# SMSD75/Timetuning

Measured on AMD Instinct MI355X. Metric: clip-frames/sec, higher is better.
Workload: dtype f32-split(f16x3); 1 GPU; C2: dino-s16 full TimeT training step (fwd+bwd+AdamW), 4-frame 224x224 clips, 32 clips/GPU, 200 prototypes; clips_per_gpu=32, num_frames=4, num_clusters=200, global_batch=32, parallelism=dp1

## Files before the change

include/timetuning_hip.h:

```cpp
#ifndef TIMETUNING_HIP_H
#define TIMETUNING_HIP_H

#include <stddef.h>
#include <stdint.h>

#ifdef __cplusplus
extern "C" {
#endif

#define TT_OK 0
#define TT_EINVAL (-1)
#define TT_ELAUNCH (-2)
#define TT_EUNSUPPORTED (-3)

typedef void* tt_stream_t;

const char* tt_last_error(void);
int tt_abi_version(void);
int tt_set_tuning_knob(const char* name, int value);
int tt_tuning_knob_info(int index, const char** name, int* default_value, int* value);
int tt_device_info(char* name, int cap);

size_t tt_linear_ksplit_workspace_bytes(void);
int tt_linear_ksplit_workspace_init(void* workspace, size_t workspace_bytes, tt_stream_t stream);
// ... 41 lines not shown
int tt_patch_embed_fwd_planes(const float* img, const int32_t* frame_map, const void* w_planes, const float* bias, const float* cls,
                              const float* pos, float* tokens, int F, int C, int H, int W, int P, int D, void* workspace,
                              size_t workspace_bytes, tt_stream_t stream);

int tt_layernorm_fwd(const float* x, const float* gamma, const float* beta, float* y, float* mean, float* rstd,
                     int rows, int D, float eps, int skip_group, tt_stream_t stream);
size_t tt_amax_slot_bytes(void);
int tt_layernorm_bwd(const float* dy, const float* x, const float* gamma, const float* mean, const float* rstd,
                     float* dx, float* dgamma, float* dbeta, int rows, int D, int add_to_dx, int skip_group,
                     void* workspace, size_t workspace_bytes, float* amax_out, tt_stream_t stream);
size_t tt_layernorm_bwd_workspace_bytes(int rows, int D);

int tt_attention_fwd(const float* qkv, float* out, float* lse, float* probs, int F, int N, int H, int hd,
                     float scale, tt_stream_t stream);
int tt_attention_bwd(const float* qkv, const float* out, const float* dout, const float* lse, float* dqkv, int F,
                     int N, int H, int hd, float scale, void* workspace, size_t workspace_bytes, float* amax_out, tt_stream_t stream);
size_t tt_attention_bwd_workspace_bytes(int F, int N, int H, int hd);
int tt_attention_bwd_bf16(const float* qkv, const float* out, const float* dout, const float* lse, float* dqkv, int F, int N, int H, int hd,
                          float scale, void* workspace, size_t workspace_bytes, tt_stream_t stream);
int tt_attention_bwd_pairs(const float* qkv, const float* out, const float* dout, const float* lse, float* dqkv, int F, int N, int H, int hd,
                           float scale, const float* dout_amax, void* workspace, size_t workspace_bytes, int* range_flag, float* amax_out,
                           tt_stream_t stream);
size_t tt_attention_bwd_pairs_workspace_bytes(int F, int N, int H, int hd);

int tt_l2norm_fwd(const float* x, int ldx, float* xn, float* inv_norm, int rows, int D, tt_stream_t stream);
int tt_l2norm_bwd(const float* dxn, const float* xn, const float* inv_norm, float* dx, int rows, int D, float* amax_out,
                  tt_stream_t stream);
int tt_normalize_rows_inplace(float* w, int rows, int D, tt_stream_t stream);

int tt_sinkhorn(const float* scores, float* q_out, int B_total, int K, int row0, int rows_out, float eps,
                int iters, void* workspace, size_t workspace_bytes, tt_stream_t stream);
size_t tt_sinkhorn_workspace_bytes(int B_total, int K);
size_t tt_sinkhorn_local_workspace_bytes(int B_loc, int K);
int tt_sinkhorn_local_begin(const float* scores, float* u_out, int B_loc, int K, float eps, void* workspace, size_t workspace_bytes,
                            tt_stream_t stream);
int tt_sinkhorn_local_step(const float* u_in, float* u_out, int B_loc, int B_total, int K, void* workspace, size_t workspace_bytes,
                           tt_stream_t stream);
int tt_sinkhorn_local_end(const float* u_in, float* q_out, int B_loc, int rows_out, int K, void* workspace, size_t workspace_bytes,
                          tt_stream_t stream);
int tt_sinkhorn_from_q(const float* Q, int transposed, float* q_out, int B_total, int K, int row0, int rows_out, int iters,
                       void* workspace, size_t workspace_bytes, tt_stream_t stream);

int tt_split_planes(const float* src, void* dst_planes, long long plane_stride, int planes, long long n, tt_stream_t stream);
int tt_layernorm_fwd_planes(const float* x, const float* gamma, const float* beta, void* y_planes, long long plane_stride,
                            int planes, float* mean, float* rstd, int rows, int D, float eps, int skip_group,
                            tt_stream_t stream);
// ... 365 lines not shown
```

timetuning_amd/_lib.py:

```python
from __future__ import annotations

import ctypes as C
import os
import subprocess

_HERE = os.path.dirname(os.path.abspath(__file__))
LIB_PATH = os.environ.get("TT_LIB_PATH") or os.path.join(_HERE, "libtimetuning_hip.so")
CSRC = os.path.join(_HERE, "csrc")

c_f32p = C.c_void_p
c_vp = C.c_void_p
c_i = C.c_int
c_ll = C.c_longlong
c_f = C.c_float
c_d = C.c_double
c_sz = C.c_size_t


class AdamwTensor(C.Structure):
    _fields_ = [("p", C.c_void_p), ("g", C.c_void_p), ("m", C.c_void_p), ("v", C.c_void_p), ("n", C.c_longlong),
                ("lr", C.c_float), ("weight_decay", C.c_float)]


class VitBlockParams(C.Structure):
# ... 57 lines not shown
    "tt_split_pairs_dual_parts": (c_i, [c_vp, c_vp, c_vp, c_vp, c_vp, c_vp, c_i, c_i, c_i, c_vp, c_sz, c_vp, c_vp]),
    "tt_transpose_pairs": (c_i, [c_vp, c_vp, c_i, c_i, c_i, c_vp]),
    "tt_linear_bwd_data_pairs": (c_i, [c_vp, c_vp, c_vp, c_vp, c_vp, c_i, c_i, c_i, c_vp, c_sz, c_vp, c_vp]),
    "tt_linear_bwd_weight_pairs_workspace_bytes": (c_sz, [c_i, c_i, c_i]),
    "tt_linear_bwd_weight_pairs": (c_i, [c_vp, c_vp, c_vp, c_vp, c_i, c_i, c_i, c_vp, c_sz, c_vp]),
    "tt_split_pairs_dual_multi": (c_i, [c_vp, c_vp, c_vp, c_vp, c_vp, c_vp, c_i, c_vp, c_vp]),
    "tt_patch_embed_pairs_workspace_bytes": (c_sz, [c_i, c_i, c_i, c_i, c_i]),
    "tt_patch_embed_fwd_pairs": (c_i, [c_vp, c_vp, c_vp, c_vp, c_vp, c_vp, c_vp, c_i, c_i, c_i, c_i, c_i, c_i, c_vp, c_sz, c_vp, c_vp]),
    "tt_linear_bwd_weight_pairs_tn_ok": (c_i, [c_i, c_i, c_i]),
    "tt_linear_bwd_weight_pairs_tn_workspace_bytes": (c_sz, [c_i, c_i, c_i]),
    "tt_linear_bwd_weight_pairs_tn": (c_i, [c_vp, c_vp, c_vp, c_vp, c_i, c_i, c_i, c_vp, c_sz, c_vp]),
    "tt_linear_bwd_weight_pairs_tn_bias": (c_i, [c_vp, c_vp, c_vp, c_vp, c_i, c_i, c_i, c_vp, c_sz, c_vp, c_i, c_vp, c_vp]),
    "tt_transpose_planes": (c_i, [c_vp, c_vp, c_i, c_i, c_i, c_vp]),
    "tt_transpose_planes_colsum_workspace_bytes": (c_sz, [c_i, c_i, c_i]),
    "tt_transpose_planes_colsum": (c_i, [c_vp, c_vp, c_i, c_i, c_i, c_vp, c_vp, c_sz, c_vp]),
    "tt_linear_bwd_data_planes": (c_i, [c_vp, c_ll, c_vp, c_ll, c_i, c_vp, c_vp, c_i, c_i, c_i, c_vp, c_sz, c_vp]),
    "tt_linear_bwd_weight_planes": (c_i, [c_vp, c_ll, c_vp, c_ll, c_i, c_vp, c_i, c_i, c_i, c_vp, c_sz, c_vp]),
    "tt_linear_bwd_weight_planes_workspace_bytes": (c_sz, [c_i, c_i, c_i]),
    "tt_attention_bwd": (c_i, [c_vp, c_vp, c_vp, c_vp, c_vp, c_i, c_i, c_i, c_i, c_f, c_vp, c_sz, c_vp, c_vp]),
    "tt_attention_bwd_workspace_bytes": (c_sz, [c_i, c_i, c_i, c_i]),
    "tt_attention_bwd_bf16": (c_i, [c_vp, c_vp, c_vp, c_vp, c_vp, c_i, c_i, c_i, c_i, c_f, c_vp, c_sz, c_vp]),
    "tt_attention_bwd_pairs": (c_i, [c_vp, c_vp, c_vp, c_vp, c_vp, c_i, c_i, c_i, c_i, c_f, c_vp, c_vp, c_sz, c_vp, c_vp, c_vp]),
    "tt_attention_bwd_pairs_workspace_bytes": (c_sz, [c_i, c_i, c_i, c_i]),
    "tt_l2norm_fwd": (c_i, [c_vp, c_i, c_vp, c_vp, c_i, c_i, c_vp]),
    "tt_l2norm_bwd": (c_i, [c_vp, c_vp, c_vp, c_vp, c_i, c_i, c_vp, c_vp]),
    "tt_normalize_rows_inplace": (c_i, [c_vp, c_i, c_i, c_vp]),
    "tt_sinkhorn": (c_i, [c_vp, c_vp, c_i, c_i, c_i, c_i, c_f, c_i, c_vp, c_sz, c_vp]),
    "tt_sinkhorn_workspace_bytes": (c_sz, [c_i, c_i]),
    "tt_sinkhorn_local_workspace_bytes": (c_sz, [c_i, c_i]),
    "tt_sinkhorn_local_begin": (c_i, [c_vp, c_vp, c_i, c_i, c_f, c_vp, c_sz, c_vp]),
    "tt_sinkhorn_local_step": (c_i, [c_vp, c_vp, c_i, c_i, c_i, c_vp, c_sz, c_vp]),
    "tt_sinkhorn_local_end": (c_i, [c_vp, c_vp, c_i, c_i, c_i, c_vp, c_sz, c_vp]),
    "tt_sinkhorn_from_q": (c_i, [c_vp, c_i, c_vp, c_i, c_i, c_i, c_i, c_i, c_vp, c_sz, c_vp]),
    "tt_label_propagate": (c_i, [c_vp, c_vp, c_vp, c_vp, c_i, c_i, c_i, c_i, c_i, c_i, c_i, c_i, c_f, c_i, c_vp, c_sz, c_vp]),
    "tt_label_propagate_workspace_bytes": (c_sz, [c_i, c_i, c_i, c_i, c_i, c_i]),
    "tt_label_propagate_route": (c_i, [c_i, c_i, c_i, c_i, c_i, c_i]),
    "tt_ce_loss_fwd_bwd": (c_i, [c_vp, c_vp, c_vp, c_vp, c_vp, c_i, c_i, c_f, c_vp, c_sz, c_vp]),
    "tt_ce_workspace_bytes": (c_sz, [c_i]),
    "tt_queue_push": (c_i, [c_vp, c_vp, c_vp, c_vp, c_i, c_i, c_i, c_vp]),
    "tt_adamw_step": (c_i, [C.POINTER(AdamwTensor), c_i, c_i, c_f, c_f, c_f, c_vp]),
    "tt_scale_tensors": (c_i, [C.POINTER(AdamwTensor), c_i, c_vp, c_vp]),
    "tt_ema_update": (c_i, [c_vp, c_vp, c_ll, c_d, c_vp]),
    "tt_vit_forward_workspace_bytes": (c_sz, [c_i, c_i, c_i, c_i, c_i]),
    "tt_vit_forward": (c_i, [C.POINTER(VitParams), c_vp, c_vp, c_i, c_i, c_i, c_i, c_vp, c_vp, c_i, c_vp, c_vp, c_vp, c_sz, c_vp]),
    "tt_mlp_head_forward_workspace_bytes": (c_sz, [c_i, C.POINTER(LinearParams), c_i]),
    "tt_mlp_head_forward": (c_i, [c_vp, c_i, C.POINTER(LinearParams), c_i, c_vp, c_i, c_vp, c_sz, c_vp]),
# ... 145 lines not shown
```

timetuning_amd/csrc/attention_bwd.hip:

```cpp
#include "common.hpp"

namespace tt {

typedef float f32x4 __attribute__((ext_vector_type(4)));
typedef __bf16 bf16x4 __attribute__((ext_vector_type(4)));
typedef short s16x4 __attribute__((ext_vector_type(4)));
typedef _Float16 f16x4 __attribute__((ext_vector_type(4)));
typedef _Float16 f16x8 __attribute__((ext_vector_type(8)));

__device__ __forceinline__ s16x4 pack_bf16(float a, float b, float c, float d) {
  const bf16x4 v = {(__bf16)a, (__bf16)b, (__bf16)c, (__bf16)d};
  return __builtin_bit_cast(s16x4, v);
}
__device__ __forceinline__ f32x4 mma_bf16(s16x4 a, s16x4 b, f32x4 acc) { return __builtin_amdgcn_mfma_f32_16x16x16bf16_1k(a, b, acc, 0, 0, 0); }

__device__ __forceinline__ bool split4(float a, float b, float c, float d, f16x4& hi, f16x4& lo) {
  _Float16 h0, l0, h1, l1, h2, l2, h3, l3;
  split_pair(a, h0, l0); split_pair(b, h1, l1); split_pair(c, h2, l2); split_pair(d, h3, l3);
  hi = (f16x4){h0, h1, h2, h3};
  lo = (f16x4){l0, l1, l2, l3};
  return pair_hi_bad(h0) || pair_hi_bad(h1) || pair_hi_bad(h2) || pair_hi_bad(h3);
}
__device__ __forceinline__ void mma_pair8(f16x8 ah, f16x8 al, f16x8 bh, f16x8 bl, f32x4& acc1, f32x4& acc2) {
  acc1 = __builtin_amdgcn_mfma_f32_16x16x32_f16(ah, bh, acc1, 0, 0, 0);
// ... 507 lines not shown
#pragma unroll
    for (int d = 0; d < 4; ++d) {
      dk[d] = fold_pair(dk[d], dk2[d], 1.0f);
      dv[d] = fold_pair(dv[d], dv2[d], 1.0f);
    }
  }
  if (wave_active && key < N) {
    float* ok_ = dqkv + ((long long)f * N + key) * D3 + D + h * BHD + 4 * g;
    float* ov = ok_ + D;
#pragma unroll
    for (int d = 0; d < 4; ++d) {
      const float4 wk_ = make_float4(dk[d][0] * scale, dk[d][1] * scale, dk[d][2] * scale, dk[d][3] * scale);
      const float4 wv_ = make_float4(dv[d][0] * vscale, dv[d][1] * vscale, dv[d][2] * vscale, dv[d][3] * vscale);
      *reinterpret_cast<float4*>(ok_ + 16 * d) = wk_;
      *reinterpret_cast<float4*>(ov + 16 * d) = wv_;
      am = fmaxf(fmaxf(am, fmaxf(fabsf(wk_.x), fabsf(wk_.y))), fmaxf(fabsf(wk_.z), fabsf(wk_.w)));
      am = fmaxf(fmaxf(am, fmaxf(fabsf(wv_.x), fabsf(wv_.y))), fmaxf(fabsf(wv_.z), fabsf(wv_.w)));
    }
  }
  if (amax_out) amax_publish(amax_out, am);
  if constexpr (PAIR) range_flag_raise(range_flag, bad);
}

}

using namespace tt;

extern "C" size_t tt_attention_bwd_workspace_bytes(int F, int N, int H, int hd) {
  (void)hd;
  return (size_t)F * H * N * sizeof(float);
}

template <bool BF16>
static int attention_bwd_impl(const float* qkv, const float* out, const float* dout, const float* lse, float* dqkv, int F, int N,
                              int H, int hd, float scale, void* workspace, size_t workspace_bytes, float* amax_out, tt_stream_t stream) {
  TT_REQUIRE(qkv && out && dout && lse && dqkv && workspace, "attention_bwd: null pointer");
  TT_REQUIRE(hd == 64, "attention_bwd: head_dim must be 64 (got %d)", hd);
  TT_REQUIRE(F > 0 && H > 0 && N > 0, "attention_bwd: bad shape");
  TT_REQUIRE(workspace_bytes >= tt_attention_bwd_workspace_bytes(F, N, H, hd), "attention_bwd: workspace too small");
  TT_REQUIRE(aligned16(qkv) && aligned16(out) && aligned16(dout) && aligned16(dqkv), "attention_bwd: buffers must be 16-byte aligned");
  hipStream_t s = as_stream(stream);
  float* delta = static_cast<float*>(workspace);
  dim3 grid(xcd_group_grid(F * H, (N + 63) / 64));
  hipLaunchKernelGGL(attention_bwd_dq_kernel<BF16>, grid, dim3(256), 0, s, qkv, out, dout, lse, dqkv, delta, amax_out, N, H, F * H, scale);
  hipLaunchKernelGGL(attention_bwd_dkv_kernel<BF16>, grid, dim3(256), 0, s, qkv, dout, lse, delta, dqkv, amax_out, N, H, F * H, scale);
  TT_CHECK_LAUNCH("attention_bwd");
// ... 17 lines not shown
  TT_REQUIRE(F > 0 && H > 0 && N > 0, "attention_bwd_pairs: bad shape");
  TT_REQUIRE(workspace_bytes >= tt_attention_bwd_pairs_workspace_bytes(F, N, H, hd), "attention_bwd_pairs: workspace too small");
  TT_REQUIRE(aligned16(qkv) && aligned16(out) && aligned16(dout) && aligned16(dqkv) && aligned16(workspace), "attention_bwd_pairs: buffers must be 16-byte aligned");
  hipStream_t s = as_stream(stream);
  float* delta = static_cast<float*>(workspace);
  const float* part = delta + (size_t)F * H * N;
  const long long n = (long long)F * N * H * hd;
  int n_part = (int)((n + 4095) / 4096 < kBwdAmaxParts ? (n + 4095) / 4096 : kBwdAmaxParts);
  if (dout_amax) {
    part = const_cast<float*>(dout_amax);
    n_part = -kAmaxWays;
  } else {
    hipLaunchKernelGGL(attention_bwd_amax_kernel, dim3(n_part), dim3(256), 0, s, dout, n, const_cast<float*>(part));
  }
  dim3 grid(xcd_group_grid(F * H, (N + 63) / 64));
  hipLaunchKernelGGL((attention_bwd_dq_kernel<false, true>), grid, dim3(256), 0, s, qkv, out, dout, lse, dqkv, delta, amax_out, N, H, F * H, scale, part, n_part,
                     range_flag);
  hipLaunchKernelGGL((attention_bwd_dkv_kernel<false, true>), grid, dim3(256), 0, s, qkv, dout, lse, delta, dqkv, amax_out, N, H, F * H, scale, part, n_part,
                     range_flag);
  TT_CHECK_LAUNCH("attention_bwd_pairs");
  return TT_OK;
}

extern "C" int tt_attention_bwd_bf16(const float* qkv, const float* out, const float* dout, const float* lse, float* dqkv, int F, int N,
                                     int H, int hd, float scale, void* workspace, size_t workspace_bytes, tt_stream_t stream) {
  return attention_bwd_impl<true>(qkv, out, dout, lse, dqkv, F, N, H, hd, scale, workspace, workspace_bytes, nullptr, stream);
}
```

timetuning_amd/engine.py:

```python
from __future__ import annotations

from typing import Dict, List, Optional

import torch

from . import hip_ops as ops

f32 = torch.float32



def _param_tag(w: torch.Tensor, kind) -> tuple:
    static = getattr(w, "_tt_static", False) and not w.requires_grad
    return (w.data_ptr(), w._version, 0 if static else ops.PARAM_EPOCH, kind)


def weight_planes(w: torch.nn.Parameter, planes: int) -> torch.Tensor:
    hit = getattr(w, "_tt_planes", None)
    tag = _param_tag(w, planes)
    if hit is None or hit[0] != tag:
        hit = (tag, ops.split_pairs(w.detach()) if planes == 2 else ops.split_planes(w.detach(), planes))
        w._tt_planes = hit
    return hit[1]

# ... 85 lines not shown
        aux["qkv"] = qkv.view(Fr, N, 3 * D)
    att, lse, _ = ops.attention_fwd(qkv.view(Fr, N, 3 * D), num_heads, save_lse=save is not None)
    x_mid = ops.linear_fwd(att.view(M, D), blk.attn.proj.weight, blk.attn.proj.bias, residual=x2d,
                           out=None if save is not None else x2d)
    if save is not None:
        h2, save["mean2"], save["rstd2"] = ops.layernorm_fwd(x_mid, blk.norm2.weight, blk.norm2.bias, save_stats=True)
        a, pre = ops.linear_fwd(h2, blk.mlp.fc1.weight, blk.mlp.fc1.bias, act=1, save_pre=True)
    else:
        h2 = ops.layernorm_fwd(x_mid, blk.norm2.weight, blk.norm2.bias, out=h1.view(M, D))
        a = ops.linear_fwd(h2, blk.mlp.fc1.weight, blk.mlp.fc1.bias, act=1)
    x_out = ops.linear_fwd(a, blk.mlp.fc2.weight, blk.mlp.fc2.bias, residual=x_mid, out=None if save is not None else x_mid)
    if save is not None:
        save.update(x_in=x, h1=h1, qkv=qkv, att=att, lse=lse, x_mid=x_mid, h2=h2, pre=pre, a=a)
    return x_out.view(Fr, N, D)


def block_forward_pairs_kept(x: torch.Tensor, blk, num_heads: int, save: dict, aux: Optional[dict] = None) -> torch.Tensor:
    Fr, N, D = x.shape
    M = Fr * N
    x2d = x.view(M, D)
    at, mlp = blk.attn, blk.mlp
    h1p, save["mean1"], save["rstd1"] = ops.layernorm_fwd_pairs(x, blk.norm1.weight, blk.norm1.bias, save_stats=True)
    if ops.attention_pairs_ok(N, D // num_heads):
        o = ops.linear_fwd_pairs(h1p, weight_planes(at.qkv.weight, 2), at.qkv.bias, out_pairs=True)
        qkv = o["y"]
        attp, att, lse = ops.attention_fwd_pairs(o["pairs"].view(Fr, N, 6 * D), num_heads, out_f32=True, save_lse=True)
        attp = attp.view(M, 2 * D)
    else:
        qkv = ops.linear_fwd_pairs(h1p, weight_planes(at.qkv.weight, 2), at.qkv.bias)["y"]
        att, lse, _ = ops.attention_fwd(qkv.view(Fr, N, 3 * D), num_heads, save_lse=True)
        attp = ops.split_pairs(att.view(M, D))
    if aux is not None:
        aux["qkv"] = qkv.view(Fr, N, 3 * D)
    x_mid = ops.linear_fwd_pairs(attp, weight_planes(at.proj.weight, 2), at.proj.bias, residual=x2d)["y"]
    h2p, save["mean2"], save["rstd2"] = ops.layernorm_fwd_pairs(x_mid, blk.norm2.weight, blk.norm2.bias, save_stats=True)
    o = ops.linear_fwd_pairs(h2p, weight_planes(mlp.fc1.weight, 2), mlp.fc1.bias, act=1, out_f32=False, out_pairs=True, save_pre=True)
    x_out = ops.linear_fwd_pairs(o["pairs"], weight_planes(mlp.fc2.weight, 2), mlp.fc2.bias, residual=x_mid)["y"]
    save.update(x_in=x, h1p=h1p, qkv=qkv, att=att, attp=attp, lse=lse, x_mid=x_mid, h2p=h2p, pre=o["pre"], ap=o["pairs"], pairs=True)
    return x_out.view(Fr, N, D)


def weight_pairs_t(w: torch.Tensor) -> torch.Tensor:
    hit = getattr(w, "_tt_pairs_t", None)
    tag = _param_tag(w, "T")
    if hit is None or hit[0] != tag:
        fwd = getattr(w, "_tt_planes", None)
        need_row = fwd is None or fwd[0] != _param_tag(w, 2)
        t, row, _ = ops.split_pairs_dual(w.detach(), want_row=need_row)
        if need_row:
            w._tt_planes = (_param_tag(w, 2), row)
        hit = (tag, t)
        w._tt_pairs_t = hit
    return hit[1]


def _bwd_both_pairs(dy: torch.Tensor, w: torch.Tensor, xp: torch.Tensor, gelu_pre: Optional[torch.Tensor] = None, need_dx: bool = True,
                    dw_out=None, db_out=None, dy_amax=None, dx_amax_out=None):
    return ops.linear_bwd_pairs(dy, weight_pairs_t(w), gelu_pre=gelu_pre, need_dx=need_dx, dw_out=dw_out, db_out=db_out, x_pairs=xp,
                                dy_amax=dy_amax, dx_amax_out=dx_amax_out if need_dx else None)


# ... 18 lines not shown

def block_backward(dx_out: torch.Tensor, blk, num_heads: int, sv: dict, f0: int, f1: int, grads: Dict[torch.nn.Parameter, torch.Tensor],
                   need_dx: bool = True, after_mlp=None, out=None, dx_out_amax=None, amax_pool=None):
    take = amax_pool.take if amax_pool is not None else (lambda: None)
    Fr, N, D = sv["x_in"].shape
    r0, r1 = f0 * N, f1 * N
    out = out or (lambda p: None)
    o = lambda lin: dict(dw_out=out(lin.weight), db_out=out(lin.bias))
    oln = lambda ln: dict(dg_out=out(ln.weight), db_out=out(ln.bias))
    if sv.get("pairs"):
        a_fc1, a_proj, a_qkv, a_in = take(), take(), take(), take()
        d_pre, grads[blk.mlp.fc2.weight], grads[blk.mlp.fc2.bias] = _bwd_both_pairs(dx_out, blk.mlp.fc2.weight, sv["ap"][r0:r1], sv["pre"][r0:r1],
                                                                                     dy_amax=dx_out_amax, dx_amax_out=a_fc1, **o(blk.mlp.fc2))
        d_h2, grads[blk.mlp.fc1.weight], grads[blk.mlp.fc1.bias] = _bwd_both_pairs(d_pre, blk.mlp.fc1.weight, sv["h2p"][r0:r1], dy_amax=a_fc1,
                                                                                    **o(blk.mlp.fc1))
        dx_mid, grads[blk.norm2.weight], grads[blk.norm2.bias] = ops.layernorm_bwd(
            d_h2, sv["x_mid"][r0:r1], blk.norm2.weight, sv["mean2"][r0:r1], sv["rstd2"][r0:r1], dx_accum=dx_out, amax_out=a_proj, **oln(blk.norm2))
        if after_mlp is not None:
            after_mlp()
        att_pairs = ops.ATTN_BWD_PAIRS and D // num_heads == 64
        a_att = take() if (att_pairs and amax_pool is not None and not ops.linear_bwd_data_pairs_is_persistent(r1 - r0, D, D)) else None
        d_att, grads[blk.attn.proj.weight], grads[blk.attn.proj.bias] = _bwd_both_pairs(dx_mid, blk.attn.proj.weight, sv["attp"][r0:r1],
                                                                                        dy_amax=a_proj, dx_amax_out=a_att, **o(blk.attn.proj))
        dqkv = ops.attention_bwd(sv["qkv"].view(Fr, N, 3 * D)[f0:f1], sv["att"][f0:f1], d_att.view(f1 - f0, N, D), sv["lse"][f0:f1], num_heads,
                                 amax_out=a_qkv, pair_products=att_pairs, dout_amax=a_att)
        d_h1, grads[blk.attn.qkv.weight], grads[blk.attn.qkv.bias] = _bwd_both_pairs(dqkv.view((f1 - f0) * N, 3 * D), blk.attn.qkv.weight,
                                                                                       sv["h1p"][r0:r1], dy_amax=a_qkv, **o(blk.attn.qkv))
        dx_in, grads[blk.norm1.weight], grads[blk.norm1.bias] = ops.layernorm_bwd(
            d_h1, sv["x_in"].view(Fr * N, D)[r0:r1], blk.norm1.weight, sv["mean1"][r0:r1], sv["rstd1"][r0:r1], dx_accum=dx_mid,
            amax_out=a_in if need_dx else None, **oln(blk.norm1))
        if amax_pool is not None:
            return (dx_in, a_in) if need_dx else (None, None)
        return dx_in if need_dx else None
    a, pre, h2 = sv["a"][r0:r1], sv["pre"][r0:r1], sv["h2"][r0:r1]
    d_pre, grads[blk.mlp.fc2.weight], grads[blk.mlp.fc2.bias] = _bwd_both(dx_out, blk.mlp.fc2.weight, a, pre, **o(blk.mlp.fc2))
    d_h2, grads[blk.mlp.fc1.weight], grads[blk.mlp.fc1.bias] = _bwd_both(d_pre, blk.mlp.fc1.weight, h2, **o(blk.mlp.fc1))
    dx_mid, grads[blk.norm2.weight], grads[blk.norm2.bias] = ops.layernorm_bwd(
        d_h2, sv["x_mid"][r0:r1], blk.norm2.weight, sv["mean2"][r0:r1], sv["rstd2"][r0:r1], dx_accum=dx_out, **oln(blk.norm2))
    if after_mlp is not None:
        after_mlp()
    att = sv["att"].view(Fr * N, D)[r0:r1]
    d_att, grads[blk.attn.proj.weight], grads[blk.attn.proj.bias] = _bwd_both(dx_mid, blk.attn.proj.weight, att, **o(blk.attn.proj))
    qkv = sv["qkv"].view(Fr, N, 3 * D)[f0:f1]
    dqkv = ops.attention_bwd(qkv, sv["att"][f0:f1], d_att.view(f1 - f0, N, D), sv["lse"][f0:f1], num_heads,
                             bf16_products=ops.plane_count() == 1 and D // num_heads == 64)
    dqkv2 = dqkv.view((f1 - f0) * N, 3 * D)
    h1 = sv["h1"].view(Fr * N, D)[r0:r1]
    d_h1, grads[blk.attn.qkv.weight], grads[blk.attn.qkv.bias] = _bwd_both(dqkv2, blk.attn.qkv.weight, h1, **o(blk.attn.qkv))
# ... 610 lines not shown
```

timetuning_amd/hip_ops.py:

```python
from __future__ import annotations

import contextlib
import ctypes as C
import os
from typing import Optional, Sequence

import numpy as np
import torch

from . import _lib

f32 = torch.float32


def _stream() -> int:
    return torch.cuda.current_stream().cuda_stream


def _p(t: Optional[torch.Tensor]):
    return None if t is None else t.data_ptr()


def _chk(t: torch.Tensor, name: str, dtype=f32) -> torch.Tensor:
    if not t.is_cuda:
# ... 444 lines not shown
    ws = _ws(nb, x.device)
    _lib.check(lib.tt_layernorm_bwd(_p(dy), _p(x), _p(gamma), _p(mean), _p(rstd), _p(dx), _p(dg), _p(db), rows, D,
                                    1 if dx_accum is not None else 0, skip, _p(ws), nb, _p(amax_out), _stream()), "tt_layernorm_bwd")
    return dx, dg, db


def attention_fwd(qkv, num_heads: int, save_lse=False, return_probs=False):
    lib = _lib.load()
    _chk(qkv, "qkv")
    F, N, D3 = qkv.shape
    D = D3 // 3
    hd = D // num_heads
    out = torch.empty((F, N, D), dtype=f32, device=qkv.device)
    lse = torch.empty((F, num_heads, N), dtype=f32, device=qkv.device) if save_lse else None
    probs = torch.empty((F, num_heads, N, N), dtype=f32, device=qkv.device) if return_probs else None
    _lib.check(lib.tt_attention_fwd(_p(qkv), _p(out), _p(lse), _p(probs), F, N, num_heads, hd, float(hd ** -0.5), _stream()),
               "tt_attention_fwd")
    return out, lse, probs


ATTN_BWD_PAIRS = os.environ.get("TT_ATTN_BWD_PAIRS", "1") != "0"


def attention_bwd(qkv, out, dout, lse, num_heads: int, bf16_products: bool = False, amax_out=None, pair_products: bool = False, dout_amax=None):
    lib = _lib.load()
    _chk(qkv, "qkv"); _chk(out, "out"); _chk(dout, "dout"); _chk(lse, "lse")
    F, N, D3 = qkv.shape
    hd = D3 // 3 // num_heads
    dqkv = torch.empty_like(qkv)
    if pair_products and not bf16_products:
        nb = lib.tt_attention_bwd_pairs_workspace_bytes(F, N, num_heads, hd)
        ws = _ws(nb, qkv.device)
        _lib.check(lib.tt_attention_bwd_pairs(_p(qkv), _p(out), _p(dout), _p(lse), _p(dqkv), F, N, num_heads, hd, float(hd ** -0.5), _p(dout_amax), _p(ws), nb,
                                              _p(range_flag(qkv.device)), _p(amax_out), _stream()), "tt_attention_bwd_pairs")
        return dqkv
    nb = lib.tt_attention_bwd_workspace_bytes(F, N, num_heads, hd)
    ws = _ws(nb, qkv.device)
    if bf16_products:
        _lib.check(lib.tt_attention_bwd_bf16(_p(qkv), _p(out), _p(dout), _p(lse), _p(dqkv), F, N, num_heads, hd, float(hd ** -0.5), _p(ws), nb, _stream()),
                   "tt_attention_bwd_bf16")
    else:
        _lib.check(lib.tt_attention_bwd(_p(qkv), _p(out), _p(dout), _p(lse), _p(dqkv), F, N, num_heads, hd, float(hd ** -0.5), _p(ws), nb, _p(amax_out),
                                        _stream()), "tt_attention_bwd")
    return dqkv



def l2norm_fwd(x, save_inv=False, out=None):
    lib = _lib.load()
    if x.dim() != 2 or x.stride(1) != 1 or not x.is_cuda or x.dtype != f32:
        raise ValueError("l2norm_fwd: expected a 2-D fp32 GPU tensor with unit inner stride")
# ... 2229 lines not shown
```

Baseline: 19250 clip-frames/sec.

## Run attention backward directly from saved fp16 qkv pair images

```diff
diff --git a/include/timetuning_hip.h b/include/timetuning_hip.h
--- a/include/timetuning_hip.h
+++ b/include/timetuning_hip.h
@@ -87,6 +87,9 @@
                            float scale, const float* dout_amax, void* workspace, size_t workspace_bytes, int* range_flag, float* amax_out,
                            tt_stream_t stream);
 size_t tt_attention_bwd_pairs_workspace_bytes(int F, int N, int H, int hd);
+int tt_attention_bwd_pairs_images(const void* qkv_pairs, const float* out, const float* dout, const float* lse, float* dqkv, int F, int N, int H,
+                                  int hd, float scale, const float* dout_amax, void* workspace, size_t workspace_bytes, int* range_flag,
+                                  float* amax_out, tt_stream_t stream);
 
 int tt_l2norm_fwd(const float* x, int ldx, float* xn, float* inv_norm, int rows, int D, tt_stream_t stream);
 int tt_l2norm_bwd(const float* dxn, const float* xn, const float* inv_norm, float* dx, int rows, int D, float* amax_out,
diff --git a/timetuning_amd/_lib.py b/timetuning_amd/_lib.py
--- a/timetuning_amd/_lib.py
+++ b/timetuning_amd/_lib.py
@@ -103,6 +103,7 @@
     "tt_attention_bwd_bf16": (c_i, [c_vp, c_vp, c_vp, c_vp, c_vp, c_i, c_i, c_i, c_i, c_f, c_vp, c_sz, c_vp]),
     "tt_attention_bwd_pairs": (c_i, [c_vp, c_vp, c_vp, c_vp, c_vp, c_i, c_i, c_i, c_i, c_f, c_vp, c_vp, c_sz, c_vp, c_vp, c_vp]),
     "tt_attention_bwd_pairs_workspace_bytes": (c_sz, [c_i, c_i, c_i, c_i]),
+    "tt_attention_bwd_pairs_images": (c_i, [c_vp, c_vp, c_vp, c_vp, c_vp, c_i, c_i, c_i, c_i, c_f, c_vp, c_vp, c_sz, c_vp, c_vp, c_vp]),
     "tt_l2norm_fwd": (c_i, [c_vp, c_i, c_vp, c_vp, c_i, c_i, c_vp]),
     "tt_l2norm_bwd": (c_i, [c_vp, c_vp, c_vp, c_vp, c_i, c_i, c_vp, c_vp]),
     "tt_normalize_rows_inplace": (c_i, [c_vp, c_i, c_i, c_vp]),
diff --git a/timetuning_amd/csrc/attention_bwd.hip b/timetuning_amd/csrc/attention_bwd.hip
--- a/timetuning_amd/csrc/attention_bwd.hip
+++ b/timetuning_amd/csrc/attention_bwd.hip
@@ -553,6 +553,341 @@
   if constexpr (PAIR) range_flag_raise(range_flag, bad);
 }
 
+constexpr int IMG_B = BCH * 256;
+#ifndef TT_ABI_DBG
+#define TT_ABI_DBG 0
+#endif
+__device__ __forceinline__ void abi_mma(f16x8 ah, f16x8 al, f16x8 bh, f16x8 bl, f32x4& acc1, f32x4& acc2, bool off) {
+  if (off) { acc1[0] += (float)ah[0] * (float)bh[0]; acc2[0] += (float)al[0] * (float)bl[0]; }
+  else mma_pair8(ah, al, bh, bl, acc1, acc2);
+}
+__device__ __forceinline__ bool abi_split8(const float* v, float s, f16x8& hi, f16x8& lo) {
+  if constexpr (TT_ABI_DBG & 4) {
+#pragma unroll
+    for (int j = 0; j < 8; ++j) { hi[j] = (_Float16)(v[j] * s); lo[j] = hi[j]; }
+    return false;
+  } else {
+    return split8(v, s, hi, lo);
+  }
+}
+__device__ __forceinline__ float abi_exp(float x) { return (TT_ABI_DBG & 4) ? x : fast_exp(x); }
+__device__ __forceinline__ int img_swz(int row) { return ((row & 3) << 2) | (((row >> 2) & 1) << 1) | ((row >> 3) & 1); }
+__device__ __forceinline__ int img_off(int row, int ch) { return row * 256 + ((ch ^ img_swz(row)) << 4); }
+typedef __attribute__((address_space(3))) void* img_lds_ptr_t;
+
+__device__ __forceinline__ void img_issue(__amdgpu_buffer_rsrc_t rsrc, unsigned row_b, int chunk, int N, unsigned char* dst, int wave, int lane) {
+  if (TT_ABI_DBG & 32) return;
+#pragma unroll
+  for (int i = 0; i < 2; ++i) {
+    const int piece = 2 * wave + i, row = piece * 4 + (lane >> 4);
+    const int key = chunk * BCH + row;
+    const unsigned off = (unsigned)(key < N ? key : N - 1) * row_b + (unsigned)(((lane & 15) ^ img_swz(row)) << 4);
+    __builtin_amdgcn_raw_ptr_buffer_load_lds(rsrc, (img_lds_ptr_t)(dst + piece * 1024), 16, off, 0, 0, 0);
+  }
+}
+__device__ __forceinline__ void img_row_frags(const unsigned char* img, int row, int g, f16x8 (&hi)[2], f16x8 (&lo)[2]) {
+#pragma unroll
+  for (int s = 0; s < 2; ++s) {
+    const int ch = 8 * (g & 1) + 2 * s + (g >> 1);
+    if constexpr (TT_ABI_DBG & 8) {
+      hi[s] = (f16x8){(_Float16)row, 1, 1, 1, 1, 1, 1, 1};
+      lo[s] = hi[s];
+      continue;
+    }
+    hi[s] = *reinterpret_cast<const f16x8*>(img + img_off(row, ch));
+    lo[s] = *reinterpret_cast<const f16x8*>(img + img_off(row, ch + 4));
+  }
+}
+__device__ __forceinline__ void pair_row_frags(const _Float16* p, int g, f16x8 (&hi)[2], f16x8 (&lo)[2]) {
+#pragma unroll
+  for (int s = 0; s < 2; ++s) {
+    const int ch = 8 * (g & 1) + 2 * s + (g >> 1);
+    hi[s] = *reinterpret_cast<const f16x8*>(p + 8 * ch);
+    lo[s] = *reinterpret_cast<const f16x8*>(p + 8 * ch + 32);
+  }
+}
+__device__ __forceinline__ void f32_row_vals(const float* p, int g, float (&r)[16]) {
+#pragma unroll
+  for (int s = 0; s < 2; ++s) {
+    const int d0 = 32 * (g & 1) + 8 * (2 * s + (g >> 1));
+    float4 a = make_float4(0.f, 0.f, 0.f, 0.f), b = a;
+    if (p) {
+      a = *reinterpret_cast<const float4*>(p + d0);
+      b = *reinterpret_cast<const float4*>(p + d0 + 4);
+    }
+    r[8 * s] = a.x; r[8 * s + 1] = a.y; r[8 * s + 2] = a.z; r[8 * s + 3] = a.w;
+    r[8 * s + 4] = b.x; r[8 * s + 5] = b.y; r[8 * s + 6] = b.z; r[8 * s + 7] = b.w;
+  }
+}
+__device__ __forceinline__ int img_tr_base(int lane) {
+  const int g = lane >> 4, q4 = (lane >> 2) & 3, p4 = lane & 3;
+  return img_off(4 * g + q4, p4 >> 1) + 8 * (p4 & 1);
+}
+__device__ __forceinline__ f16x8 img_tr_frag(const unsigned char* img, int tr_base, int c0) {
+  union { s16x4 s2[2]; f16x8 v; } u;
+  if constexpr (TT_ABI_DBG & 16) return (f16x8){(_Float16)c0, 1, 1, 1, 1, 1, 1, 1};
+  const unsigned char* p = img + (tr_base ^ (c0 << 4));
+  u.s2[0] = __builtin_amdgcn_ds_read_tr16_b64_v4i16((s16x4 __attribute__((address_space(3)))*)(p));
+  u.s2[1] = __builtin_amdgcn_ds_read_tr16_b64_v4i16((s16x4 __attribute__((address_space(3)))*)(p + 16 * 256));
+  return u.v;
+}
+
+__global__ __launch_bounds__(256, 3) void attention_bwd_dq_images_kernel(const _Float16* __restrict__ qkvp, const float* __restrict__ out,
+                                                                         const float* __restrict__ dout, const float* __restrict__ lse,
+                                                                         float* __restrict__ dqkv, float* __restrict__ delta,
+                                                                         float* __restrict__ amax_out, int N, int H, int FH, float scale,
+                                                                         const float* __restrict__ amax_part, int n_part, int* range_flag) {
+  __shared__ __attribute__((aligned(16))) unsigned char smem[4 * IMG_B];
+  __shared__ float sred[4];
+  const float S = bwd_grad_scale(amax_part, n_part, sred);
+  bool bad = false;
+  const int tid = threadIdx.x, lane = tid & 63, qi = lane & 15, g = lane >> 4;
+  const int wave = __builtin_amdgcn_readfirstlane(tid >> 6);
+  int fh, tile64;
+  if (!xcd_group_decode(blockIdx.x, (N + 63) / 64, FH, fh, tile64)) return;
+  const int f = fh / H, h = fh - f * H, D = H * BHD, D3 = 3 * D;
+  const long long RS = 6ll * D;
+  const _Float16* pbase = qkvp + (long long)f * N * RS + h * 128;
+  const unsigned row_b = (unsigned)RS * 2u;
+  const __amdgpu_buffer_rsrc_t rk = __builtin_amdgcn_make_buffer_rsrc(const_cast<_Float16*>(pbase + 2 * D), 0, 0x7fffffff, 0x00020000);
+  const __amdgpu_buffer_rsrc_t rv = __builtin_amdgcn_make_buffer_rsrc(const_cast<_Float16*>(pbase + 4 * D), 0, 0x7fffffff, 0x00020000);
+  auto issue = [&](int chunk, int buf) {
+    img_issue(rk, row_b, chunk, N, smem + buf * 2 * IMG_B, wave, lane);
+    img_issue(rv, row_b, chunk, N, smem + buf * 2 * IMG_B + IMG_B, wave, lane);
+  };
+  const int nchunks = (N + BCH - 1) / BCH;
+  issue(0, 0);
+  const int q0 = tile64 * 64, q = q0 + wave * 16 + qi;
+  const bool wave_active = q0 + wave * 16 < N;
+
+  f16x8 qh[2], ql[2], doh[2], dol[2];
+  float dl = 0.f;
+  {
+    float doreg[16], oreg[16];
+    pair_row_frags(pbase + (long long)(q < N ? q : N - 1) * RS, g, qh, ql);
+    f32_row_vals(q < N ? dout + ((long long)f * N + q) * D + h * BHD : nullptr, g, doreg);
+    f32_row_vals(q < N ? out + ((long long)f * N + q) * D + h * BHD : nullptr, g, oreg);
+#pragma unroll
+    for (int s = 0; s < 16; ++s) dl += doreg[s] * oreg[s];
+#pragma unroll
+    for (int t = 0; t < 2; ++t) bad |= split8(doreg + 8 * t, S, doh[t], dol[t]);
+  }
+  dl += __shfl_xor(dl, 16, 64);
+  dl += __shfl_xor(dl, 32, 64);
+  const float inv_s = 1.0f / S;
+  const float S2 = S * 0.000244140625f;
+  const float lse_q = (q < N) ? lse[((long long)f * H + h) * N + q] : 0.f;
+  if (q < N && g == 0) delta[((long long)f * H + h) * N + q] = dl;
+  const int tr_base = img_tr_base(lane);
+
+  f32x4 dq[4], dq2[4];
+#pragma unroll
+  for (int d = 0; d < 4; ++d) {
+    dq[d] = (f32x4){0.f, 0.f, 0.f, 0.f};
+    dq2[d] = (f32x4){0.f, 0.f, 0.f, 0.f};
+  }
+  for (int c = 0; c < nchunks; ++c) {
+    const int buf = c & 1;
+    asm volatile("s_waitcnt vmcnt(0)" ::: "memory");
+    __syncthreads();
+    if (c + 1 < nchunks) issue(c + 1, buf ^ 1);
+    if (wave_active) {
+      const unsigned char* Ki = smem + buf * 2 * IMG_B;
+      const unsigned char* Vi = Ki + IMG_B;
+      float ds_all[8];
+#pragma unroll
+      for (int t2 = 0; t2 < 2; ++t2) {
+        f16x8 ah[2], al[2], bh[2], bl[2];
+        img_row_frags(Ki, 16 * t2 + qi, g, ah, al);
+        img_row_frags(Vi, 16 * t2 + qi, g, bh, bl);
+        f32x4 sa = (f32x4){0.f, 0.f, 0.f, 0.f}, dp = sa, sa2 = sa, dp2 = sa;
+#pragma unroll
+        for (int t = 0; t < 2; ++t) {
+          abi_mma(ah[t], al[t], qh[t], ql[t], sa, sa2, TT_ABI_DBG & 1);
+          abi_mma(bh[t], bl[t], doh[t], dol[t], dp, dp2, TT_ABI_DBG & 1);
+        }
+        sa = fold_pair(sa, sa2, scale);
+        dp = fold_pair(dp, dp2, inv_s);
+#pragma unroll
+        for (int e = 0; e < 4; ++e) {
+          const int key = c * BCH + 16 * t2 + 4 * g + e;
+          const float p = (key < N && q < N) ? abi_exp(sa[e] - lse_q) : 0.f;
+          ds_all[4 * t2 + e] = p * (dp[e] - dl);
+        }
+      }
+      f16x8 dsh, dsl;
+      bad |= abi_split8(ds_all, S2, dsh, dsl);
+#pragma unroll
+      for (int d = 0; d < 4; ++d) {
+        const int c0 = 8 * (d >> 1) + 2 * (d & 1);
+        abi_mma(img_tr_frag(Ki, tr_base, c0), img_tr_frag(Ki, tr_base, c0 + 4), dsh, dsl, dq[d], dq2[d], TT_ABI_DBG & 2);
+      }
+    }
+  }
+  float am = 0.f;
+  scale /= S2;
+#pragma unroll
+  for (int d = 0; d < 4; ++d) dq[d] = fold_pair(dq[d], dq2[d], 1.0f);
+  if (wave_active && q < N) {
+    float* o = dqkv + ((long long)f * N + q) * D3 + h * BHD + 4 * g;
+#pragma unroll
+    for (int d = 0; d < 4; ++d) {
+      const float4 w = make_float4(dq[d][0] * scale, dq[d][1] * scale, dq[d][2] * scale, dq[d][3] * scale);
+      *reinterpret_cast<float4*>(o + 16 * d) = w;
+      am = fmaxf(fmaxf(am, fmaxf(fabsf(w.x), fabsf(w.y))), fmaxf(fabsf(w.z), fabsf(w.w)));
+    }
+  }
+  if (amax_out) amax_publish(amax_out, am);
+  range_flag_raise(range_flag, bad);
+}
+
+__global__ __launch_bounds__(256, 2) void attention_bwd_dkv_images_kernel(const _Float16* __restrict__ qkvp, const float* __restrict__ dout,
+                                                                          const float* __restrict__ lse, const float* __restrict__ delta,
+                                                                          float* __restrict__ dqkv, float* __restrict__ amax_out, int N, int H,
+                                                                          int FH, float scale, const float* __restrict__ amax_part, int n_part,
+                                                                          int* range_flag) {
+  __shared__ __attribute__((aligned(16))) unsigned char smem[4 * IMG_B];
+  __shared__ float Ls[2 * BCH], Dl[2 * BCH];
+  __shared__ float sred[4];
+  const float S = bwd_grad_scale(amax_part, n_part, sred);
+  bool bad = false;
+  const int tid = threadIdx.x, lane = tid & 63, ki = lane & 15, g = lane >> 4;
+  const int wave = __builtin_amdgcn_readfirstlane(tid >> 6);
+  int fh, tile64;
+  if (!xcd_group_decode(blockIdx.x, (N + 63) / 64, FH, fh, tile64)) return;
+  const int f = fh / H, h = fh - f * H, D = H * BHD, D3 = 3 * D;
+  const long long RS = 6ll * D;
+  const _Float16* pbase = qkvp + (long long)f * N * RS + h * 128;
+  const unsigned row_b = (unsigned)RS * 2u;
+  const __amdgpu_buffer_rsrc_t rq = __builtin_amdgcn_make_buffer_rsrc(const_cast<_Float16*>(pbase), 0, 0x7fffffff, 0x00020000);
+  const float* dob = dout + (long long)f * N * D + h * BHD;
+  const int k0 = tile64 * 64, key = k0 + wave * 16 + ki;
+  const bool wave_active = k0 + wave * 16 < N;
+
+  float4 sto[2];
+  float stl = 0.f, std_ = 0.f;
+  auto gload = [&](int chunk) {
+#pragma unroll
+    for (int i = 0; i < 2; ++i) {
+      const int u = tid + 256 * i, row = u >> 4, c4 = (u & 15) * 4;
+      const int q = chunk * BCH + row;
+      sto[i] = make_float4(0.f, 0.f, 0.f, 0.f);
+      if (q < N) sto[i] = *reinterpret_cast<const float4*>(dob + (long long)q * D + c4);
+    }
+    if (tid < BCH) {
+      const int q = chunk * BCH + tid;
+      stl = (q < N) ? lse[((long long)f * H + h) * N + q] : 0.f;
+      std_ = (q < N) ? delta[((long long)f * H + h) * N + q] : 0.f;
+    }
+  };
+  auto swrite = [&](int buf) {
+    unsigned char* Oi = smem + buf * 2 * IMG_B + IMG_B;
+#pragma unroll
+    for (int i = 0; i < 2; ++i) {
+      const int u = tid + 256 * i, row = u >> 4, c4 = (u & 15) * 4;
+      f16x4 hh, ll;
+      bad |= split4(sto[i].x * S, sto[i].y * S, sto[i].z * S, sto[i].w * S, hh, ll);
+      const int ch = 8 * (c4 >> 5) + ((c4 & 31) >> 3), at = (c4 & 7) * 2;
+      *reinterpret_cast<f16x4*>(Oi + img_off(row, ch) + at) = hh;
+      *reinterpret_cast<f16x4*>(Oi + img_off(row, ch + 4) + at) = ll;
+    }
+    if (tid < BCH) {
+      Ls[buf * BCH + tid] = stl;
+      Dl[buf * BCH + tid] = std_;
+    }
+  };
+  const int nchunks = (N + BCH - 1) / BCH;
+  img_issue(rq, row_b, 0, N, smem, wave, lane);
+  gload(0);
+
+  f16x8 kh[2], kl[2], vh[2], vl[2];
+  {
+    const _Float16* prow = pbase + (long long)(key < N ? key : N - 1) * RS;
+    pair_row_frags(prow + 2 * D, g, kh, kl);
+    pair_row_frags(prow + 4 * D, g, vh, vl);
+  }
+  const float inv_s = 1.0f / S;
+  const float S2 = S * 0.000244140625f;
+  const int tr_base = img_tr_base(lane);
+
+  f32x4 dk[4], dv[4], dk2[4], dv2[4];
+#pragma unroll
+  for (int d = 0; d < 4; ++d) {
+    dk[d] = (f32x4){0.f, 0.f, 0.f, 0.f};
+    dv[d] = dk[d]; dk2[d] = dk[d]; dv2[d] = dk[d];
+  }
+  swrite(0);
+  for (int c = 0; c < nchunks; ++c) {
+    const int buf = c & 1;
+    asm volatile("s_waitcnt vmcnt(0)" ::: "memory");
+    __syncthreads();
+    if (c + 1 < nchunks) {
+      img_issue(rq, row_b, c + 1, N, smem + (buf ^ 1) * 2 * IMG_B, wave, lane);
+      gload(c + 1);
+    }
+    if (wave_active) {
+      const unsigned char* Qi = smem + buf * 2 * IMG_B;
+      const unsigned char* Oi = Qi + IMG_B;
+      float p_all[8], ds_all[8];
+#pragma unroll
+      for (int t2 = 0; t2 < 2; ++t2) {
+        f16x8 ah[2], al[2], bh[2], bl[2];
+        img_row_frags(Qi, 16 * t2 + ki, g, ah, al);
+        img_row_frags(Oi, 16 * t2 + ki, g, bh, bl);
+        f32x4 sa = (f32x4){0.f, 0.f, 0.f, 0.f}, dp = sa, sa2 = sa, dp2 = sa;
+#pragma unroll
+        for (int t = 0; t < 2; ++t) {
+          abi_mma(ah[t], al[t], kh[t], kl[t], sa, sa2, TT_ABI_DBG & 1);
+          abi_mma(bh[t], bl[t], vh[t], vl[t], dp, dp2, TT_ABI_DBG & 1);
+        }
+        sa = fold_pair(sa, sa2, scale);
+        dp = fold_pair(dp, dp2, inv_s);
+#pragma unroll
+        for (int e = 0; e < 4; ++e) {
+          const int ql = 16 * t2 + 4 * g + e;
+          const bool ok = (c * BCH + ql < N) && (key < N);
+          const float p = ok ? abi_exp(sa[e] - Ls[buf * BCH + ql]) : 0.f;
+          p_all[4 * t2 + e] = p;
+          ds_all[4 * t2 + e] = p * (dp[e] - Dl[buf * BCH + ql]);
+        }
+      }
+      f16x8 ph, pl, dsh, dsl;
+      abi_split8(p_all, 1.0f, ph, pl);
+      bad |= abi_split8(ds_all, S2, dsh, dsl);
+#pragma unroll
+      for (int d = 0; d < 4; ++d) {
+        const int c0 = 8 * (d >> 1) + 2 * (d & 1);
+        abi_mma(img_tr_frag(Oi, tr_base, c0), img_tr_frag(Oi, tr_base, c0 + 4), ph, pl, dv[d], dv2[d], TT_ABI_DBG & 2);
+        abi_mma(img_tr_frag(Qi, tr_base, c0), img_tr_frag(Qi, tr_base, c0 + 4), dsh, dsl, dk[d], dk2[d], TT_ABI_DBG & 2);
+      }
+    }
+    if (c + 1 < nchunks) swrite(buf ^ 1);
+  }
+  float am = 0.f;
+  scale /= S2;
+  const float vscale = inv_s;
+#pragma unroll
+  for (int d = 0; d < 4; ++d) {
+    dk[d] = fold_pair(dk[d], dk2[d], 1.0f);
+    dv[d] = fold_pair(dv[d], dv2[d], 1.0f);
+  }
+  if (wave_active && key < N) {
+    float* ok_ = dqkv + ((long long)f * N + key) * D3 + D + h * BHD + 4 * g;
+    float* ov = ok_ + D;
+#pragma unroll
+    for (int d = 0; d < 4; ++d) {
+      const float4 wk_ = make_float4(dk[d][0] * scale, dk[d][1] * scale, dk[d][2] * scale, dk[d][3] * scale);
+      const float4 wv_ = make_float4(dv[d][0] * vscale, dv[d][1] * vscale, dv[d][2] * vscale, dv[d][3] * vscale);
+      *reinterpret_cast<float4*>(ok_ + 16 * d) = wk_;
+      *reinterpret_cast<float4*>(ov + 16 * d) = wv_;
+      am = fmaxf(fmaxf(am, fmaxf(fabsf(wk_.x), fabsf(wk_.y))), fmaxf(fabsf(wk_.z), fabsf(wk_.w)));
+      am = fmaxf(fmaxf(am, fmaxf(fabsf(wv_.x), fabsf(wv_.y))), fmaxf(fabsf(wv_.z), fabsf(wv_.w)));
+    }
+  }
+  if (amax_out) amax_publish(amax_out, am);
+  range_flag_raise(range_flag, bad);
+}
+
 }
 
 using namespace tt;
@@ -616,6 +951,37 @@
   return TT_OK;
 }
 
+extern "C" int tt_attention_bwd_pairs_images(const void* qkv_pairs, const float* out, const float* dout, const float* lse, float* dqkv, int F, int N, int H,
+                                             int hd, float scale, const float* dout_amax, void* workspace, size_t workspace_bytes, int* range_flag,
+                                             float* amax_out, tt_stream_t stream) {
+  TT_REQUIRE(qkv_pairs && out && dout && lse && dqkv && workspace, "attention_bwd_pairs_images: null pointer");
+  TT_REQUIRE(hd == 64, "attention_bwd_pairs_images: head_dim must be 64 (got %d)", hd);
+  TT_REQUIRE(F > 0 && H > 0 && N > 0, "attention_bwd_pairs_images: bad shape");
+  TT_REQUIRE(((long long)N + 1) * H * 64 * 12 < 0x7fffffffLL, "attention_bwd_pairs_images: a frame's pair image must stay under 2 GB");
+  TT_REQUIRE(workspace_bytes >= tt_attention_bwd_pairs_workspace_bytes(F, N, H, hd), "attention_bwd_pairs_images: workspace too small");
+  TT_REQUIRE(aligned16(qkv_pairs) && aligned16(out) && aligned16(dout) && aligned16(dqkv) && aligned16(workspace),
+             "attention_bwd_pairs_images: buffers must be 16-byte aligned");
+  hipStream_t s = as_stream(stream);
+  float* delta = static_cast<float*>(workspace);
+  const float* part = delta + (size_t)F * H * N;
+  const long long n = (long long)F * N * H * hd;
+  int n_part = (int)((n + 4095) / 4096 < kBwdAmaxParts ? (n + 4095) / 4096 : kBwdAmaxParts);
+  if (dout_amax) {
+    part = dout_amax;
+    n_part = -kAmaxWays;
+  } else {
+    hipLaunchKernelGGL(attention_bwd_amax_kernel, dim3(n_part), dim3(256), 0, s, dout, n, const_cast<float*>(part));
+  }
+  const _Float16* qp = static_cast<const _Float16*>(qkv_pairs);
+  dim3 grid(xcd_group_grid(F * H, (N + 63) / 64));
+  hipLaunchKernelGGL(attention_bwd_dq_images_kernel, grid, dim3(256), 0, s, qp, out, dout, lse, dqkv, delta, amax_out, N, H, F * H, scale, part, n_part,
+                     range_flag);
+  hipLaunchKernelGGL(attention_bwd_dkv_images_kernel, grid, dim3(256), 0, s, qp, dout, lse, delta, dqkv, amax_out, N, H, F * H, scale, part, n_part,
+                     range_flag);
+  TT_CHECK_LAUNCH("attention_bwd_pairs_images");
+  return TT_OK;
+}
+
 extern "C" int tt_attention_bwd_bf16(const float* qkv, const float* out, const float* dout, const float* lse, float* dqkv, int F, int N,
                                      int H, int hd, float scale, void* workspace, size_t workspace_bytes, tt_stream_t stream) {
   return attention_bwd_impl<true>(qkv, out, dout, lse, dqkv, F, N, H, hd, scale, workspace, workspace_bytes, nullptr, stream);
diff --git a/timetuning_amd/engine.py b/timetuning_amd/engine.py
--- a/timetuning_amd/engine.py
+++ b/timetuning_amd/engine.py
@@ -131,12 +131,13 @@
     at, mlp = blk.attn, blk.mlp
     h1p, save["mean1"], save["rstd1"] = ops.layernorm_fwd_pairs(x, blk.norm1.weight, blk.norm1.bias, save_stats=True)
     if ops.attention_pairs_ok(N, D // num_heads):
-        o = ops.linear_fwd_pairs(h1p, weight_planes(at.qkv.weight, 2), at.qkv.bias, out_pairs=True)
-        qkv = o["y"]
-        attp, att, lse = ops.attention_fwd_pairs(o["pairs"].view(Fr, N, 6 * D), num_heads, out_f32=True, save_lse=True)
+        images = ops.ATTN_BWD_PAIRS and ops.ATTN_BWD_IMAGES and D // num_heads == 64
+        o = ops.linear_fwd_pairs(h1p, weight_planes(at.qkv.weight, 2), at.qkv.bias, out_f32=aux is not None or not images, out_pairs=True)
+        qkv, qkvp = o["y"], o["pairs"].view(Fr, N, 6 * D)
+        attp, att, lse = ops.attention_fwd_pairs(qkvp, num_heads, out_f32=True, save_lse=True)
         attp = attp.view(M, 2 * D)
     else:
-        qkv = ops.linear_fwd_pairs(h1p, weight_planes(at.qkv.weight, 2), at.qkv.bias)["y"]
+        qkv, qkvp = ops.linear_fwd_pairs(h1p, weight_planes(at.qkv.weight, 2), at.qkv.bias)["y"], None
         att, lse, _ = ops.attention_fwd(qkv.view(Fr, N, 3 * D), num_heads, save_lse=True)
         attp = ops.split_pairs(att.view(M, D))
     if aux is not None:
@@ -145,7 +146,7 @@
     h2p, save["mean2"], save["rstd2"] = ops.layernorm_fwd_pairs(x_mid, blk.norm2.weight, blk.norm2.bias, save_stats=True)
     o = ops.linear_fwd_pairs(h2p, weight_planes(mlp.fc1.weight, 2), mlp.fc1.bias, act=1, out_f32=False, out_pairs=True, save_pre=True)
     x_out = ops.linear_fwd_pairs(o["pairs"], weight_planes(mlp.fc2.weight, 2), mlp.fc2.bias, residual=x_mid)["y"]
-    save.update(x_in=x, h1p=h1p, qkv=qkv, att=att, attp=attp, lse=lse, x_mid=x_mid, h2p=h2p, pre=o["pre"], ap=o["pairs"], pairs=True)
+    save.update(x_in=x, h1p=h1p, qkv=qkv, qkvp=qkvp, att=att, attp=attp, lse=lse, x_mid=x_mid, h2p=h2p, pre=o["pre"], ap=o["pairs"], pairs=True)
     return x_out.view(Fr, N, D)
 
 
@@ -210,8 +211,10 @@
         a_att = take() if (att_pairs and amax_pool is not None and not ops.linear_bwd_data_pairs_is_persistent(r1 - r0, D, D)) else None
         d_att, grads[blk.attn.proj.weight], grads[blk.attn.proj.bias] = _bwd_both_pairs(dx_mid, blk.attn.proj.weight, sv["attp"][r0:r1],
                                                                                         dy_amax=a_proj, dx_amax_out=a_att, **o(blk.attn.proj))
-        dqkv = ops.attention_bwd(sv["qkv"].view(Fr, N, 3 * D)[f0:f1], sv["att"][f0:f1], d_att.view(f1 - f0, N, D), sv["lse"][f0:f1], num_heads,
-                                 amax_out=a_qkv, pair_products=att_pairs, dout_amax=a_att)
+        qkv32, qkvp = sv["qkv"], sv.get("qkvp")
+        dqkv = ops.attention_bwd(qkv32.view(Fr, N, 3 * D)[f0:f1] if qkv32 is not None else None, sv["att"][f0:f1], d_att.view(f1 - f0, N, D),
+                                 sv["lse"][f0:f1], num_heads, amax_out=a_qkv, pair_products=att_pairs, dout_amax=a_att,
+                                 qkv_pairs=qkvp[f0:f1] if qkvp is not None else None)
         d_h1, grads[blk.attn.qkv.weight], grads[blk.attn.qkv.bias] = _bwd_both_pairs(dqkv.view((f1 - f0) * N, 3 * D), blk.attn.qkv.weight,
                                                                                        sv["h1p"][r0:r1], dy_amax=a_qkv, **o(blk.attn.qkv))
         dx_in, grads[blk.norm1.weight], grads[blk.norm1.bias] = ops.layernorm_bwd(
diff --git a/timetuning_amd/hip_ops.py b/timetuning_amd/hip_ops.py
--- a/timetuning_amd/hip_ops.py
+++ b/timetuning_amd/hip_ops.py
@@ -490,11 +490,28 @@
 ATTN_BWD_PAIRS = os.environ.get("TT_ATTN_BWD_PAIRS", "1") != "0"
 
 
-def attention_bwd(qkv, out, dout, lse, num_heads: int, bf16_products: bool = False, amax_out=None, pair_products: bool = False, dout_amax=None):
-    lib = _lib.load()
-    _chk(qkv, "qkv"); _chk(out, "out"); _chk(dout, "dout"); _chk(lse, "lse")
-    F, N, D3 = qkv.shape
-    hd = D3 // 3 // num_heads
+ATTN_BWD_IMAGES = os.environ.get("TT_ATTN_BWD_IMAGES", "1") != "0"
+
+
+def attention_bwd(qkv, out, dout, lse, num_heads: int, bf16_products: bool = False, amax_out=None, pair_products: bool = False, dout_amax=None,
+                  qkv_pairs=None):
+    lib = _lib.load()
+    _chk(out, "out"); _chk(dout, "dout"); _chk(lse, "lse")
+    F, N, D = out.shape
+    hd = D // num_heads
+    if qkv_pairs is not None and pair_products and not bf16_products and hd == 64 and (ATTN_BWD_IMAGES or qkv is None):
+        if not (qkv_pairs.is_cuda and qkv_pairs.dtype == f16 and qkv_pairs.is_contiguous() and tuple(qkv_pairs.shape) == (F, N, 6 * D)):
+            raise ValueError("attention_bwd: qkv_pairs must be a contiguous fp16 GPU tensor [F, N, 6 D]")
+        dqkv = torch.empty((F, N, 3 * D), dtype=f32, device=out.device)
+        nb = lib.tt_attention_bwd_pairs_workspace_bytes(F, N, num_heads, hd)
+        ws = _ws(nb, out.device)
+        _lib.check(lib.tt_attention_bwd_pairs_images(_p(qkv_pairs), _p(out), _p(dout), _p(lse), _p(dqkv), F, N, num_heads, hd, float(hd ** -0.5),
+                                                     _p(dout_amax), _p(ws), nb, _p(range_flag(out.device)), _p(amax_out), _stream()),
+                   "tt_attention_bwd_pairs_images")
+        return dqkv
+    if qkv is None:
+        raise ValueError("attention_bwd: the fp32 qkv is required on this route (no pair images: head_dim != 64 or not the pair products)")
+    _chk(qkv, "qkv")
     dqkv = torch.empty_like(qkv)
     if pair_products and not bf16_products:
         nb = lib.tt_attention_bwd_pairs_workspace_bytes(F, N, num_heads, hd)
```

New measurement: 19420 clip-frames/sec, median of 6. About the same (+0.9%).
